# ruanjinchen/Point-Cloud-Flow-Matching

Measured on AMD Instinct MI355X. Metric: train-step points/sec (B=8, N=20000, xyz+rgb) at 1/2/4/8 MI355X; Chamfer ms, higher is better.
Workload: dtype fp32 ContextNet (scatter/gather ops fp32; Conv3d + 1x1 convs as bf16x3 split-operand matrix-core products, fp32 accumulate, ~2^-16 per product vs the reference's default cuDNN TF32 2^-11) + bf16 autocast per-point MLP head (reference AMP config; its per-cloud B-row layers -- embeddings, FiLM affines

## Files before the change

### point-cloud-flow-matching_amd/csrc/head_film.hip

```cpp
#include <algorithm>

#include "pcfm_common.hpp"

namespace pcfm {
namespace {

#ifndef PCFM_FILM_BWD_WPE
#define PCFM_FILM_BWD_WPE 0
#endif
#if PCFM_FILM_BWD_WPE > 0
#define FILM_BWD_ATTR __attribute__((amdgpu_waves_per_eu(PCFM_FILM_BWD_WPE)))
#else
#define FILM_BWD_ATTR
#endif
constexpr int kRowsPerBlock = 256;
constexpr int kSums = 5;

__device__ __forceinline__ float bf2f(uint32_t b) { return __uint_as_float(b << 16); }
__device__ __forceinline__ uint32_t f2bf(float x) {
  return (uint32_t)__builtin_bit_cast(uint16_t, (__bf16)x);
}

__device__ __forceinline__ float wave_sum(float x) {
#pragma unroll
  for (int off = 32; off > 0; off >>= 1) x += __shfl_xor(x, off, 64);
  return x;
}

template <int NV>
__device__ __forceinline__ void ld_f32(const float* __restrict__ p, int lane, float (&v)[NV][4]) {
#pragma unroll
  for (int j = 0; j < NV; ++j) {
    const float4 f = *reinterpret_cast<const float4*>(p + 256 * j + 4 * lane);
    v[j][0] = f.x;
    v[j][1] = f.y;
    v[j][2] = f.z;
    v[j][3] = f.w;
  }
}

template <int NV>
__device__ __forceinline__ void ld_bf16(const uint16_t* __restrict__ p, int lane,
                                        float (&v)[NV][4]) {
#pragma unroll
  for (int j = 0; j < NV; ++j) {
    const uint2 q = *reinterpret_cast<const uint2*>(p + 256 * j + 4 * lane);
    v[j][0] = bf2f(q.x & 0xFFFFu);
    v[j][1] = bf2f(q.x >> 16);
    v[j][2] = bf2f(q.y & 0xFFFFu);
    v[j][3] = bf2f(q.y >> 16);
  }
}

template <int NV>
__device__ __forceinline__ void st_f32(float* __restrict__ p, int lane, const float (&v)[NV][4]) {
#pragma unroll
  for (int j = 0; j < NV; ++j)
    *reinterpret_cast<float4*>(p + 256 * j + 4 * lane) =
        make_float4(v[j][0], v[j][1], v[j][2], v[j][3]);
}

template <int NV>
__device__ __forceinline__ void st_bf16(uint16_t* __restrict__ p, int lane,
                                        const float (&v)[NV][4]) {
#pragma unroll
  for (int j = 0; j < NV; ++j) {
    uint2 q;
    q.x = f2bf(v[j][0]) | (f2bf(v[j][1]) << 16);
    q.y = f2bf(v[j][2]) | (f2bf(v[j][3]) << 16);
// ... 163 lines not shown
                       sh[j][e];
      }
#pragma unroll
      for (int j = 0; j < NV; ++j)
#pragma unroll
        for (int e = 0; e < 4; ++e) {
          const float d = du[j][e] + da[j][e] * dsilu(uu[j][e]);
          const float xc = rstd * (x[j][e] - mean);
          const float y = __builtin_fmaf(gm[j][e], xc, bt[j][e]);
          const float dy = d * sp[j][e];
          acc[0][j][e] += d * y;
          acc[1][j][e] += d;
          acc[2][j][e] += dy * xc;
          acc[3][j][e] += dy;
          xh[j][e] = xc;
          dxh[j][e] = dy * gm[j][e];
          s1 += dxh[j][e];
          s2 += dxh[j][e] * xc;
        }
      const float m1 = wave_sum(s1) * (1.0f / W), m2 = wave_sum(s2) * (1.0f / W);
#pragma unroll
      for (int j = 0; j < NV; ++j)
#pragma unroll
        for (int e = 0; e < 4; ++e) g[j][e] = rstd * (dxh[j][e] - m1 - xh[j][e] * m2);
    } else {
#pragma unroll
      for (int j = 0; j < NV; ++j)
#pragma unroll
        for (int e = 0; e < 4; ++e) g[j][e] = da[j][e] * dsilu(x[j][e]);
    }
    if (dh != nullptr) st_f32<NV>(dh + off, lane, g);
    st_bf16<NV>(dh16 + off, lane, g);
#pragma unroll
    for (int j = 0; j < NV; ++j)
#pragma unroll
      for (int e = 0; e < 4; ++e) acc[4][j][e] += bf2f(f2bf(g[j][e]));
  }
  __syncthreads();
#pragma unroll
  for (int k = 0; k < kSums; ++k)
#pragma unroll
    for (int j = 0; j < NV; ++j)
#pragma unroll
      for (int e = 0; e < 4; ++e) red[wave][k][256 * j + 4 * lane + e] = acc[k][j][e];
  __syncthreads();
  float* pb = part + ((size_t)b * gridDim.x + blockIdx.x) * kSums * W;
  for (int idx = threadIdx.x; idx < kSums * W; idx += 256) {
    const int k = idx / W, c = idx - k * W;
    pb[idx] = ((red[0][k][c] + red[1][k][c]) + red[2][k][c]) + red[3][k][c];
  }
}

__global__ void __launch_bounds__(256)
    film_bwd_reduce_kernel(const float* __restrict__ part, int B, int chunks, int W,
                           float* __restrict__ dsp1, float* __restrict__ dshift,
                           float* __restrict__ perb) {
  __shared__ float red[4][64];
  const int cl = threadIdx.x & 63, grp = threadIdx.x >> 6;
  const int c = blockIdx.x * 64 + cl, k = blockIdx.y, b = blockIdx.z;
  float s = 0.0f;
  if (c < W) {
    const float* p = part + ((size_t)b * chunks * kSums + k) * W + c;
    int q = grp;
    for (; q + 12 < chunks; q += 16) {
      float v[4];
#pragma unroll
      for (int u = 0; u < 4; ++u) v[u] = p[(size_t)(q + 4 * u) * kSums * W];
#pragma unroll
      for (int u = 0; u < 4; ++u) s += v[u];
    }
    for (; q < chunks; q += 4) s += p[(size_t)q * kSums * W];
  }
  red[grp][cl] = s;
  __syncthreads();
  if (grp != 0 || c >= W) return;
  s = ((red[0][cl] + red[1][cl]) + red[2][cl]) + red[3][cl];
  float* out = k == 0 ? dsp1 : k == 1 ? dshift : perb + (size_t)(k - 2) * B * W;
  if (out != nullptr) out[(size_t)b * W + c] = s;
}

__global__ void __launch_bounds__(64)
    film_bwd_reduce2_kernel(const float* __restrict__ perb, int B, int W,
                            float* __restrict__ dgamma, float* __restrict__ dbeta,
                            float* __restrict__ dbias) {
  const int c = blockIdx.x * 64 + threadIdx.x, k = blockIdx.y;
  float* out = k == 0 ? dgamma : k == 1 ? dbeta : dbias;
  if (c >= W || out == nullptr) return;
  float s = 0.0f;
  for (int b = 0; b < B; ++b) s += perb[((size_t)k * B + b) * W + c];
  out[c] = s;
}

int film_fwd_rows() {
  const char* e = getenv("PCFM_FILM_FWD_ROWS");
  const int v = e != nullptr ? atoi(e) : 32;
  return v >= 4 && v % 4 == 0 ? v : 32;
}

bool film_ok(int b, int n, int w) {
  return b > 0 && n > 0 && (w == 256 || w == 512) &&
         (long long)b * n * w < (1LL << 40);
}

template <bool FILM>
int launch_fwd(const void* h16, const float* uprev, const void* gprev, const float* gamma,
               const float* beta, const void* sp1, const void* shift, const float* hbias, int b,
               int n, int w, float eps, float* u, void* a, float* mean, float* rstd,
               hipStream_t st) {
  const int rpb = film_fwd_rows();
  const dim3 grid(ceil_div(n, rpb), b), blk(256);
  const uint16_t* H = (const uint16_t*)h16;
  const uint16_t* G = (const uint16_t*)gprev;
  const uint16_t* S1 = (const uint16_t*)sp1;
  const uint16_t* SH = (const uint16_t*)shift;
  uint16_t* A = (uint16_t*)a;
  switch (w) {
    case 256:
      hipLaunchKernelGGL((film_fwd_kernel<1, FILM>), grid, blk, 0, st, H, uprev, G, gamma, beta,
                         S1, SH, hbias, n, eps, u, A, mean, rstd, rpb);
      break;
    default:
      hipLaunchKernelGGL((film_fwd_kernel<2, FILM>), grid, blk, 0, st, H, uprev, G, gamma, beta,
                         S1, SH, hbias, n, eps, u, A, mean, rstd, rpb);
  }
  return check_launch(FILM ? "head_film_fwd" : "head_silu_fwd");
}

template <bool FILM>
int launch_bwd(const float* dhn, const void* da16, const float* u, const void* h16,
               const float* uprev, const void* gprev, const float* mean, const float* rstd,
               const float* gamma, const float* beta, const void* sp1, const void* shift,
               const float* hbias, int b, int n, int w, float* dh, void* dh16, float* dsp1, float* dshift, float* dgamma,
               float* dbeta, float* dbias, float* dbias_b, void* ws, hipStream_t st) {
  const int chunks = ceil_div(n, kRowsPerBlock);
  const dim3 grid(chunks, b), blk(256);
  const uint16_t* DA = (const uint16_t*)da16;
  const uint16_t* H = (const uint16_t*)h16;
  const uint16_t* G = (const uint16_t*)gprev;
  const uint16_t* S1 = (const uint16_t*)sp1;
  const uint16_t* SH = (const uint16_t*)shift;
  uint16_t* D16 = (uint16_t*)dh16;
  float* part = (float*)ws;
  switch (w) {
    case 256:
      hipLaunchKernelGGL((film_bwd_kernel<1, FILM>), grid, blk, 0, st, dhn, DA, u, H, uprev, G,
                         mean, rstd, gamma, beta, S1, SH, hbias, n, dh, D16, part);
      break;
    default:
      hipLaunchKernelGGL((film_bwd_kernel<2, FILM>), grid, blk, 0, st, dhn, DA, u, H, uprev, G,
                         mean, rstd, gamma, beta, S1, SH, hbias, n, dh, D16, part);
  }
  float* perb = part + (size_t)b * chunks * kSums * w;
  hipLaunchKernelGGL(film_bwd_reduce_kernel, dim3(ceil_div(w, 64), kSums, b), dim3(256), 0, st,
                     (const float*)part, b, chunks, w, dsp1, dshift, perb);
  hipLaunchKernelGGL(film_bwd_reduce2_kernel, dim3(ceil_div(w, 64), 3), dim3(64), 0, st,
                     (const float*)perb, b, w, dgamma, dbeta, dbias);
  if (dbias_b != nullptr) {
    const hipError_t e = hipMemcpyAsync(dbias_b, perb + 2 * (size_t)b * w,
                                        (size_t)b * w * sizeof(float), hipMemcpyDeviceToDevice, st);
    if (e != hipSuccess) {
      set_error("head_film_bwd: hipMemcpyAsync: %s", hipGetErrorString(e));
      return (int)e;
    }
  }
  return check_launch(FILM ? "head_film_bwd" : "head_silu_bwd");
}

}
}

using namespace pcfm;

extern "C" int pcfm_head_film_fwd(const void* h16, const float* hbias, const float* uprev,
                                  const void* gprev, const float* gamma, const float* beta,
                                  const void* sp1, const void* shift, int b, int n, int w,
                                  float eps, float* u, void* a, float* mean, float* rstd,
                                  void* stream) {
  PCFM_CHECK_ARG(film_ok(b, n, w), "head_film_fwd: bad shape b=%d n=%d w=%d", b, n, w);
  PCFM_CHECK_ARG(h16 != nullptr || (uprev != nullptr && gprev != nullptr),
                 "head_film_fwd: need h16 or (uprev, gprev)");
  return launch_fwd<true>(h16, uprev, gprev, gamma, beta, sp1, shift,
                          h16 != nullptr ? hbias : nullptr, b, n, w, eps, u, a, mean, rstd,
                          (hipStream_t)stream);
}

extern "C" int pcfm_head_silu_fwd(const float* uprev, const void* gprev, int b, int n, int w,
                                  void* a, void* stream) {
  PCFM_CHECK_ARG(film_ok(b, n, w), "head_silu_fwd: bad shape b=%d n=%d w=%d", b, n, w);
  return launch_fwd<false>(nullptr, uprev, gprev, nullptr, nullptr, nullptr, nullptr, nullptr, b,
                           n, w, 0.0f, nullptr, a, nullptr, nullptr, (hipStream_t)stream);
}

extern "C" size_t pcfm_head_bwd_workspace_bytes(int b, int n, int w) {
  if (!film_ok(b, n, w)) return 0;
  return ((size_t)b * ceil_div(n, kRowsPerBlock) * kSums + 3 * (size_t)b) * w * sizeof(float);
}

extern "C" int pcfm_head_film_bwd(const float* dh_next, const void* da16, const float* u,
                                  const void* h16, const float* hbias, const float* uprev,
                                  const void* gprev, const float* mean, const float* rstd,
                                  const float* gamma, const float* beta, const void* sp1,
                                  const void* shift, int b, int n, int w, float* dh, void* dh16,
                                  float* dsp1, float* dshift,
                                  float* dgamma, float* dbeta, float* dbias, float* dbias_b,
                                  void* ws, size_t ws_bytes, void* stream) {
  PCFM_CHECK_ARG(film_ok(b, n, w), "head_film_bwd: bad shape b=%d n=%d w=%d", b, n, w);
  PCFM_CHECK_ARG(h16 != nullptr || (uprev != nullptr && gprev != nullptr),
                 "head_film_bwd: need h16 or (uprev, gprev)");
  PCFM_CHECK_ARG(u != nullptr || shift != nullptr, "head_film_bwd: need u or shift");
  PCFM_CHECK_ARG(ws_bytes >= pcfm_head_bwd_workspace_bytes(b, n, w),
                 "head_film_bwd: workspace %zu < %zu bytes", ws_bytes,
                 pcfm_head_bwd_workspace_bytes(b, n, w));
  return launch_bwd<true>(dh_next, da16, u, h16, uprev, gprev, mean, rstd, gamma, beta, sp1, shift,
                          h16 != nullptr ? hbias : nullptr, b, n, w, dh, dh16, dsp1, dshift,
                          dgamma, dbeta, dbias, dbias_b, ws, (hipStream_t)stream);
}

extern "C" int pcfm_head_silu_bwd(const void* da16, const float* uprev, const void* gprev, int b,
                                  int n, int w, float* dh, void* dh16, float* dbias, void* ws,
                                  size_t ws_bytes, void* stream) {
  PCFM_CHECK_ARG(film_ok(b, n, w), "head_silu_bwd: bad shape b=%d n=%d w=%d", b, n, w);
  PCFM_CHECK_ARG(ws_bytes >= pcfm_head_bwd_workspace_bytes(b, n, w),
                 "head_silu_bwd: workspace %zu < %zu bytes", ws_bytes,
                 pcfm_head_bwd_workspace_bytes(b, n, w));
  return launch_bwd<false>(nullptr, da16, nullptr, nullptr, uprev, gprev, nullptr, nullptr,
                           nullptr, nullptr, nullptr, nullptr, nullptr, b, n, w, dh, dh16, nullptr,
                           nullptr, nullptr, nullptr, dbias, nullptr, ws, (hipStream_t)stream);
}
```

### point-cloud-flow-matching_amd/pcfm/_lib.py

```python
from __future__ import annotations

import ctypes
import os
import threading

_HERE = os.path.dirname(os.path.abspath(__file__))
LIB_PATH = os.path.join(os.path.dirname(_HERE), "csrc", "libpcfm_hip.so")
LIB_PATH = os.environ.get("PCFM_LIB", LIB_PATH)

_P = ctypes.c_void_p
_I = ctypes.c_int
_F = ctypes.c_float
_Z = ctypes.c_size_t
_L = ctypes.c_longlong
_D = ctypes.c_double
_DP = ctypes.POINTER(ctypes.c_double)

SIGNATURES = {
    "pcfm_abi_version": (_I, []),
    "pcfm_last_error": (ctypes.c_char_p, []),
    "pcfm_avg_voxelize_fwd_workspace_bytes": (_Z, [_I, _I, _I, _I]),
    "pcfm_avg_voxelize_fwd": (_I, [_P, _P, _I, _I, _I, _I, _P, _P, _P, _P, _Z, _P]),
    "pcfm_avg_voxelize_bwd": (_I, [_P, _P, _P, _I, _I, _I, _I, _P, _P]),
    "pcfm_trilinear_devoxelize_fwd": (_I, [_P, _P, _I, _I, _I, _I, _I, _P, _P, _P, _P]),
# ... 89 lines not shown
                             _P]),
    "pcfm_bn_act_fwd_split": (_I, [_P, _P, _P, _I, _I, _I, _F, _F, _F, _P, _P, _P, _P, _P, _P,
                                   _P, _Z, _P]),
    "pcfm_bn_act_bwd_split_workspace_bytes": (_Z, [_I, _I, _I]),
    "pcfm_bn_act_bwd_split": (_I, [_P, _P, _P, _P, _P, _P, _I, _I, _I, _F, _P, _P, _P, _P, _P,
                                   _Z, _P]),
    "pcfm_gn_film_workspace_bytes": (_Z, [_I, _I, _I, _I]),
    "pcfm_gn_film_res_fwd": (_I, [_P, _P, _P, _P, _P, _I, _I, _I, _I, _F, _P, _P, _P, _P, _Z,
                                  _P]),
    "pcfm_gn_film_res_bwd": (_I, [_P, _P, _P, _P, _P, _P, _P, _I, _I, _I, _I, _P, _P, _P, _P,
                                  _P, _P, _Z, _P]),
    "pcfm_debug_devox_verify_bn": (_I, [_P, _P, _P, _P, _P, _P, _F, _P, _P, _P, _P, _P, _P, _F,
                                        _P, _P, _P, _I, _I, _I, _I, _P, _P]),
    "pcfm_gn_film_res_fwd_bnin": (_I, [_P, _P, _P, _P, _P, _F, _P, _P, _P, _P, _I, _I, _I, _I,
                                       _F, _P, _P, _P, _P, _Z, _P]),
    "pcfm_gn_bnin_parts": (_I, [_I, _I]),
    "pcfm_gn_film_res_bwd_bnin": (_I, [_P, _P, _P, _P, _P, _P, _F, _P, _P, _P, _P, _P, _I, _I,
                                       _I, _I, _P, _P, _P, _P, _P, _P, _P, _Z, _P]),
    "pcfm_bn_act_bwd_apply_parts": (_I, [_P, _P, _P, _P, _P, _P, _P, _I, _I, _I, _I, _F, _P, _P,
                                         _P, _P, _P, _Z, _P]),
    "pcfm_seg_plan_bytes": (_Z, [_I, _I, _I, _I]),
    "pcfm_seg_apply_workspace_bytes": (_Z, [_I, _I, _I, _I, _I]),
    "pcfm_avg_voxelize_plan": (_I, [_P, _I, _I, _I, _P, _P, _P, _Z, _P]),
    "pcfm_avg_voxelize_fwd_planned": (_I, [_P, _P, _I, _I, _I, _I, _P, _P, _Z, _P]),
    "pcfm_trilinear_devoxelize_bwd_plan": (_I, [_P, _P, _I, _I, _I, _P, _Z, _P]),
    "pcfm_trilinear_devoxelize_bwd_planned": (_I, [_P, _P, _I, _I, _I, _I, _P, _P, _Z, _P]),
    "pcfm_adamw_chunk_elems": (_I, []),
    "pcfm_adamw_workspace_bytes": (_Z, [_I]),
    "pcfm_adamw_grad_norm": (_I, [_P, _I, _P, _I, _P, _F, _P, _P, _P, _Z, _P]),
    "pcfm_adamw_ema_step": (_I, [_P, _P, _I, _P, _P, _I, _DP, _DP, _D, _D, _D, _D, _P]),
}

ABI_VERSION = 20

ND_SIGNATURES = {
    "pcfm_chamfer_nd_abi_version": (_I, []),
    "pcfm_chamfer_nd_supported": (_I, [_I]),
    "pcfm_chamfer_nd_workspace_bytes": (_Z, [_I, _I, _I, _I]),
    "pcfm_chamfer_nd_fwd": (_I, [_P, _P, _I, _I, _I, _I, _P, _P, _P, _P, _P, _Z, _P]),
    "pcfm_chamfer_nd_bwd": (_I, [_P, _P, _I, _I, _I, _I, _P, _P, _P, _P, _P, _P, _P]),
}

ND_ABI_VERSION = 1

CROSS_SIGNATURES = {
    "pcfm_chamfer_cross_abi_version": (_I, []),
    "pcfm_chamfer_cross_supported": (_I, [_I]),
    "pcfm_chamfer_cross_workspace_bytes": (_Z, [_I, _I, _I, _I, _I]),
    "pcfm_chamfer_cross_fwd": (_I, [_P, _P, _I, _I, _I, _I, _I, _P, _P, _P, _Z, _P]),
}

CROSS_ABI_VERSION = 1

_lock = threading.Lock()
_lib = None


class PcfmError(RuntimeError):
    """A pcfm_* entry point returned a non-zero status."""


def load() -> ctypes.CDLL:
    global _lib
    if _lib is not None:
        return _lib
    with _lock:
        if _lib is None:
            if not os.path.exists(LIB_PATH):
                raise RuntimeError(
                    f"pcfm: HIP library {LIB_PATH} is not built; run "
                    "`python -c 'import __graft_entry__ as g; g.build()'` "
                    "(HIP tensors have no fallback)")
            lib = ctypes.CDLL(LIB_PATH)
            for table in (SIGNATURES, ND_SIGNATURES, CROSS_SIGNATURES):
                for name, (res, args) in table.items():
                    fn = getattr(lib, name)
                    fn.restype = res
                    fn.argtypes = args
            v = lib.pcfm_abi_version()
            if v != ABI_VERSION:
                raise RuntimeError(f"pcfm: ABI version {v} != expected {ABI_VERSION}; rebuild")
            v = lib.pcfm_chamfer_nd_abi_version()
            if v != ND_ABI_VERSION:
                raise RuntimeError(f"pcfm: chamfer_nd ABI version {v} != expected "
                                   f"{ND_ABI_VERSION}; rebuild")
            v = lib.pcfm_chamfer_cross_abi_version()
            if v != CROSS_ABI_VERSION:
                raise RuntimeError(f"pcfm: chamfer_cross ABI version {v} != expected "
                                   f"{CROSS_ABI_VERSION}; rebuild")
            _lib = lib
    return _lib


def call(name: str, *args) -> None:
    lib = load()
    rc = getattr(lib, name)(*args)
    if rc != 0:
        msg = lib.pcfm_last_error().decode(errors="replace")
        raise PcfmError(f"{name} failed (status {rc}): {msg}")


def query(name: str, *args) -> int:
    return int(getattr(load(), name)(*args))
```

### point-cloud-flow-matching_amd/pcfm/layers.py

```python
from __future__ import annotations

import os

import torch
import torch.nn as nn
import torch.nn.functional as F

__all__ = ["RowsLinear"]


class _RowsLinearBF16(torch.autograd.Function):
    @staticmethod
    def forward(ctx, x, w, b):
        ctx.save_for_backward(x, w)
        ctx.has_bias = b is not None
        return F.linear(x, w, b)

    @staticmethod
    def backward(ctx, gy):
        from pcfm import ops
        x, w = ctx.saved_tensors
        lead = gy.shape[:-1]
        g2 = gy.reshape(-1, gy.shape[-1])
        if g2.stride(1) != 1:
            g2 = g2.contiguous()
        gx = gw = gb = None
        if ctx.needs_input_grad[0]:
            gx = torch.mm(g2, w).view(*lead, w.shape[1])
        if ctx.needs_input_grad[1]:
            x2 = x.reshape(-1, x.shape[-1])
            if x2.stride(1) != 1:
                x2 = x2.contiguous()
            gw = ops.rows_wgrad_bf16(g2, x2)
        if ctx.has_bias and ctx.needs_input_grad[2]:
            gb = ops.rows_colsum(g2).to(g2.dtype) if ops.colsum_ok(g2) else g2.sum(0)
        return gx, gw, gb


class RowsLinear(nn.Linear):

    def forward(self, x: torch.Tensor) -> torch.Tensor:
        if (x.is_cuda and torch.is_autocast_enabled("cuda")
                and torch.get_autocast_dtype("cuda") == torch.bfloat16
                and x.numel() // max(1, x.shape[-1]) >= 4096):
            dt = torch.bfloat16
            b = self.bias.to(dt) if self.bias is not None else None
            with torch.autocast("cuda", enabled=False):
                return _RowsLinearBF16.apply(x.to(dt), self.weight.to(dt), b)
        return super().forward(x)


_PER_BLOCK = 6


class _HeadTrunkBF16(torch.autograd.Function):
    @staticmethod
    def forward(ctx, n, eps, x16, w_in, hb, w_out, b_out, *blk):
        from pcfm import ops
        nb = len(blk) // _PER_BLOCK
        h1 = F.linear(x16, w_in)
        hb = hb.contiguous()
        us, gs, as_, stats = [], [], [], []
        u = g = None
        for k in range(nb):
            lw, lb, sp1, sh, wk, bk = blk[_PER_BLOCK * k:_PER_BLOCK * (k + 1)]
            u, a, mean, rstd = ops.head_film_fwd(h1 if k == 0 else None, u, g, lw, lb, sp1, sh,
                                                 n, eps, hbias=hb if k == 0 else None)
            g = F.linear(a, wk, bk)
            us.append(u)
            gs.append(g)
            as_.append(a)
            stats += [mean, rstd]
        a_out = ops.head_silu_fwd(u, g, n)
        out = F.linear(a_out, w_out, b_out)
        ctx.n, ctx.eps, ctx.nb = n, eps, nb
        ctx.save_for_backward(x16, w_in, h1, hb, w_out, a_out, *us, *gs, *as_, *stats, *blk)
        return out

    @staticmethod
    def backward(ctx, gout):
        from pcfm import ops
        n, nb = ctx.n, ctx.nb
        sv = ctx.saved_tensors
        x16, w_in, h1, hb, w_out, a_out = sv[:6]
        us, gs, as_ = sv[6:6 + nb], sv[6 + nb:6 + 2 * nb], sv[6 + 2 * nb:6 + 3 * nb]
        stats = sv[6 + 3 * nb:6 + 5 * nb]
        blk = sv[6 + 5 * nb:]
        gout = gout.contiguous()
        d_w_out = ops.rows_wgrad_bf16(gout, a_out)
        d_b_out = ops.rows_colsum(gout).to(gout.dtype) if ops.colsum_ok(gout) else gout.sum(0)
        da = torch.mm(gout, w_out)
        dh, dh16, dbias = ops.head_silu_bwd(da, us[-1], gs[-1], n)
        d_blk = [None] * len(blk)
        for k in range(nb - 1, -1, -1):
            lw, lb, sp1, sh, wk, _ = blk[_PER_BLOCK * k:_PER_BLOCK * (k + 1)]
            d_blk[_PER_BLOCK * k + 4] = ops.rows_wgrad_bf16(dh16, as_[k])
            d_blk[_PER_BLOCK * k + 5] = dbias.to(torch.bfloat16)
            da = torch.mm(dh16, wk)
            first = k == 0
            res = ops.head_film_bwd(
                dh, da, None, h1 if first else None, None if first else us[k - 1],
                None if first else gs[k - 1], stats[2 * k], stats[2 * k + 1], lw, lb, sp1, n,
                want_dh=not first, hbias=hb if first else None, shift=sh)
            dh, dh16, dsp1, dshift, dgamma, dbeta, dbias = res[:7]
            if first:
                d_hb = res[7]
            d_blk[_PER_BLOCK * k] = dgamma
            d_blk[_PER_BLOCK * k + 1] = dbeta
            d_blk[_PER_BLOCK * k + 2] = dsp1.to(torch.bfloat16)
            d_blk[_PER_BLOCK * k + 3] = dshift.to(torch.bfloat16)
        d_w_in = ops.rows_wgrad_bf16(dh16, x16)
        dx = torch.mm(dh16, w_in)
        return (None, None, dx, d_w_in, d_hb, d_w_out, d_b_out, *d_blk)


def fused_trunk_supported(trunk, h: torch.Tensor, emb: torch.Tensor, n: int) -> bool:
    if not (h.is_cuda and h.dim() == 2 and torch.is_autocast_enabled("cuda")
            and torch.get_autocast_dtype("cuda") == torch.bfloat16):
        return False
    if getattr(trunk, "film_per_point", False) or emb.dim() != 2 or emb.shape[0] * n != h.shape[0]:
        return False
    width = trunk.input.out_features
    if len(trunk.films) == 0 or width not in (256, 512) or trunk.input.bias is None or trunk.out[1].bias is None:
        return False
    for seq, film in zip(trunk.blocks, trunk.films):
        norm = film.norm
        if not (isinstance(norm, nn.LayerNorm) and norm.elementwise_affine
                and norm.weight is not None and norm.bias is not None
                and tuple(norm.normalized_shape) == (width,)) or seq[1].bias is None:
            return False
    eps = {film.norm.eps for film in trunk.films}
    return len(eps) <= 1


_FILM_BATCH = os.environ.get("PCFM_FILM_BATCH", "1") != "0"


def fused_trunk(trunk, h: torch.Tensor, emb: torch.Tensor, n: int) -> torch.Tensor:
    dt = torch.bfloat16
    blk = []
    from pcfm.models import _batch_fp32
    ctx, fp32 = _batch_fp32(emb)
    nb = len(trunk.films)
    if fp32 and nb > 1 and _FILM_BATCH:
        with ctx:
# ... 57 lines not shown
```

### point-cloud-flow-matching_amd/pcfm/ops.py

```python
from __future__ import annotations

import ctypes
import types

import torch

from . import _lib, cpu_ops


def _check_cuda(x: torch.Tensor, name: str) -> None:
    if not (isinstance(x, torch.Tensor) and x.is_cuda):
        raise RuntimeError(f"{name} must be a CUDA tensor")


def _check_contig(x: torch.Tensor, name: str) -> None:
    if not x.is_contiguous():
        raise RuntimeError(f"{name} must be a contiguous tensor")


def _check_float(x: torch.Tensor, name: str) -> None:
    if x.dtype != torch.float32:
        raise RuntimeError(f"{name} must be a float tensor")


# ... 1042 lines not shown
        _lib.call("pcfm_head_film_fwd", _p(h16), _p(hbias), _p(uprev), _p(gprev), _p(gamma),
                  _p(beta),
                  _p(sp1), _p(shift), b, n, w, float(eps), _p(u), _p(a), _p(mean), _p(rstd),
                  _stream(ref))
    return u, a, mean, rstd


def head_silu_fwd(uprev, gprev, n: int):
    rows, w = uprev.shape
    a = torch.empty((rows, w), dtype=torch.bfloat16, device=uprev.device)
    _lib.call("pcfm_head_silu_fwd", _p(uprev), _p(gprev), rows // n, n, w, _p(a),
              _stream(uprev))
    return a


def head_film_bwd(dh_next, da16, u, h16, uprev, gprev, mean, rstd, gamma, beta, sp1, n: int,
                  want_dh: bool, hbias=None, shift=None):
    rows, w = da16.shape
    b = rows // n
    dev = da16.device
    dh = torch.empty((rows, w), dtype=torch.float32, device=dev) if want_dh else None
    dh16 = torch.empty((rows, w), dtype=torch.bfloat16, device=dev)
    small = torch.empty((3 * b + 3, w), dtype=torch.float32, device=dev)
    dsp1, dshift = small[:b], small[b:2 * b]
    dgamma, dbeta, dbias = small[2 * b], small[2 * b + 1], small[2 * b + 2]
    dbias_b = small[2 * b + 3:] if hbias is not None else None
    ws = _workspace(_lib.query("pcfm_head_bwd_workspace_bytes", b, n, w), da16)
    if u is None and shift is None:
        raise ValueError("head_film_bwd: need u or shift")
    with _timed("head_film_bwd", rows * w * (4 + 2 + (4 if u is not None else 0)
                                             + (2 if h16 is not None else 6)
                                             + (4 if want_dh else 0) + 2), da16):
        _lib.call("pcfm_head_film_bwd", _p(dh_next), _p(da16), _p(u), _p(h16), _p(hbias),
                  _p(uprev), _p(gprev), _p(mean), _p(rstd), _p(gamma), _p(beta), _p(sp1),
                  _p(shift), b, n,
                  w, _p(dh), _p(dh16), _p(dsp1), _p(dshift), _p(dgamma), _p(dbeta), _p(dbias),
                  _p(dbias_b), _p(ws), ws.numel(), _stream(da16))
    if hbias is not None:
        return dh, dh16, dsp1, dshift, dgamma, dbeta, dbias, dbias_b
    return dh, dh16, dsp1, dshift, dgamma, dbeta, dbias


def head_silu_bwd(da16, uprev, gprev, n: int):
    rows, w = da16.shape
    b = rows // n
    dev = da16.device
    dh = torch.empty((rows, w), dtype=torch.float32, device=dev)
    dh16 = torch.empty((rows, w), dtype=torch.bfloat16, device=dev)
    dbias = torch.empty((w,), dtype=torch.float32, device=dev)
    ws = _workspace(_lib.query("pcfm_head_bwd_workspace_bytes", b, n, w), da16)
    _lib.call("pcfm_head_silu_bwd", _p(da16), _p(uprev), _p(gprev), b, n, w, _p(dh), _p(dh16),
              _p(dbias), _p(ws), ws.numel(), _stream(da16))
    return dh, dh16, dbias


def _counter(t, like: torch.Tensor):
    if t is None:
        return None
    if t.dtype != torch.int64 or t.numel() != 1 or t.device != like.device:
        raise RuntimeError("num_batches_tracked: expected a one-element int64 tensor on the "
                           "input's device")
    return t


def bn_act_forward(x: torch.Tensor, weight: torch.Tensor, bias: torch.Tensor, eps: float,
                   slope: float, momentum: float, running_mean, running_var,
                   num_batches_tracked=None):
    _check(x, "input", "f")
    b, c = x.shape[0], x.shape[1]
    s = x.numel() // max(1, b * c)
    y = torch.empty_like(x)
    stats = torch.empty((2, c), dtype=torch.float32, device=x.device)
    ws = _workspace(_lib.query("pcfm_bn_workspace_bytes", b, c, s), x)
    with _timed("bn_act_fwd", 4 * 3 * x.numel(), x):
        _lib.call("pcfm_bn_act_fwd", _ptr(x), _ptr(weight), _ptr(bias), b, c, s, float(eps),
                  float(slope), float(momentum), _p(running_mean), _p(running_var),
                  _p(_counter(num_batches_tracked, x)), _ptr(y),
                  _ptr(stats[0]), _ptr(stats[1]), _ptr(ws), ws.numel(), _stream(x))
    return y, stats[0], stats[1]


def bn_act_forward_parts(x: torch.Tensor, stats: torch.Tensor, weight: torch.Tensor,
                         bias: torch.Tensor, eps: float, slope: float, momentum: float,
                         running_mean, running_var, num_batches_tracked=None):
    _check(x, "input", "f")
    _check(stats, "stats", "f")
    b, c = x.shape[0], x.shape[1]
    s = x.numel() // max(1, b * c)
    y = torch.empty_like(x)
    out = torch.empty((2, c), dtype=torch.float32, device=x.device)
    with _timed("bn_act_fwd", 4 * 2 * x.numel(), x):
        _lib.call("pcfm_bn_act_fwd_parts", _ptr(x), _ptr(stats), int(stats.shape[1]),
                  _ptr(weight), _ptr(bias), b, c, s, float(eps), float(slope), float(momentum),
                  _p(running_mean), _p(running_var), _p(_counter(num_batches_tracked, x)),
                  _ptr(y), _ptr(out[0]), _ptr(out[1]), _stream(x))
    return y, out[0], out[1]


def bn_act_forward_split(x: torch.Tensor, weight: torch.Tensor, bias: torch.Tensor, eps: float,
                         slope: float, momentum: float, running_mean, running_var,
                         num_batches_tracked=None):
    _check(x, "input", "f")
    b, c, r = x.shape[0], x.shape[1], x.shape[2]
    s = x.numel() // max(1, b * c)
    n = _lib.query("pcfm_conv3d_split_bytes", b, c, r)
    if n == 0 or c % 64 != 0:
# ... 320 lines not shown
```

Baseline: 5.712 million.

## Fuse head SiLU with narrow output linear in forward and backward kernels

Adds HIP kernels that compute SiLU of the last trunk activation and apply the small (up to 8 outputs) output linear in one pass, using cross-lane permlane/DPP reductions. The backward fuses the grad of the output linear (dW, db, da) with the SiLU backward and the bias column sum. The existing two-stage reduction is generalised to a variable number of sums. This avoids materialising the bf16 activation a_out, the separate GEMM launches, and the extra wgrad/colsum passes. In exchange it adds per-kind partial workspaces and a more register-heavy backward kernel.

Result: no change. 5.751 million (median of 6 runs) (+0.7%).

```diff
diff --git a/include/pcfm_head_out.h b/include/pcfm_head_out.h
--- /dev/null
+++ b/include/pcfm_head_out.h
@@ -0,0 +1,30 @@
+#ifndef PCFM_HEAD_OUT_H
+#define PCFM_HEAD_OUT_H
+
+#include <stddef.h>
+
+#ifdef __cplusplus
+extern "C" {
+#endif
+
+#define PCFM_HEAD_OUT_ABI_VERSION 1
+#define PCFM_HEAD_OUT_MAX 8
+
+int pcfm_head_out_abi_version(void);
+
+int pcfm_head_silu_out_fwd(const float* uprev, const void* gprev, const void* w_out,
+                           const void* b_out, int b, int n, int w, int n_out, void* out,
+                           void* stream);
+
+size_t pcfm_head_silu_out_bwd_workspace_bytes(int b, int n, int w, int n_out);
+
+int pcfm_head_silu_out_bwd(const void* gout, const float* uprev, const void* gprev,
+                           const void* w_out, int b, int n, int w, int n_out, float* dh,
+                           void* dh16, float* dw, float* db, float* dbias, void* ws,
+                           size_t ws_bytes, void* stream);
+
+#ifdef __cplusplus
+}
+#endif
+
+#endif
diff --git a/point-cloud-flow-matching_amd/csrc/head_film.hip b/point-cloud-flow-matching_amd/csrc/head_film.hip
--- a/point-cloud-flow-matching_amd/csrc/head_film.hip
+++ b/point-cloud-flow-matching_amd/csrc/head_film.hip
@@ -1,5 +1,6 @@
 #include <algorithm>
 
+#include "../../include/pcfm_head_out.h"
 #include "pcfm_common.hpp"
 
 namespace pcfm {
@@ -15,6 +16,8 @@
 #endif
 constexpr int kRowsPerBlock = 256;
 constexpr int kSums = 5;
+constexpr int kOutMax = PCFM_HEAD_OUT_MAX;
+constexpr int kMaxKinds = kOutMax + 2;
 
 __device__ __forceinline__ float bf2f(uint32_t b) { return __uint_as_float(b << 16); }
 __device__ __forceinline__ uint32_t f2bf(float x) {
@@ -284,43 +287,229 @@
 }
 
 __global__ void __launch_bounds__(256)
-    film_bwd_reduce_kernel(const float* __restrict__ part, int B, int chunks, int W,
-                           float* __restrict__ dsp1, float* __restrict__ dshift,
+    film_bwd_reduce_kernel(const float* __restrict__ part, int B, int chunks, int W, int nk,
+                           int nb, float* __restrict__ dsp1, float* __restrict__ dshift,
                            float* __restrict__ perb) {
   __shared__ float red[4][64];
   const int cl = threadIdx.x & 63, grp = threadIdx.x >> 6;
   const int c = blockIdx.x * 64 + cl, k = blockIdx.y, b = blockIdx.z;
+  const size_t step = (size_t)nk * W;
   float s = 0.0f;
   if (c < W) {
-    const float* p = part + ((size_t)b * chunks * kSums + k) * W + c;
+    const float* p = part + ((size_t)b * chunks * nk + k) * W + c;
     int q = grp;
     for (; q + 12 < chunks; q += 16) {
       float v[4];
 #pragma unroll
-      for (int u = 0; u < 4; ++u) v[u] = p[(size_t)(q + 4 * u) * kSums * W];
+      for (int u = 0; u < 4; ++u) v[u] = p[(size_t)(q + 4 * u) * step];
 #pragma unroll
       for (int u = 0; u < 4; ++u) s += v[u];
     }
-    for (; q < chunks; q += 4) s += p[(size_t)q * kSums * W];
+    for (; q < chunks; q += 4) s += p[(size_t)q * step];
   }
   red[grp][cl] = s;
   __syncthreads();
   if (grp != 0 || c >= W) return;
   s = ((red[0][cl] + red[1][cl]) + red[2][cl]) + red[3][cl];
-  float* out = k == 0 ? dsp1 : k == 1 ? dshift : perb + (size_t)(k - 2) * B * W;
+  float* out = k >= nb ? perb + (size_t)(k - nb) * B * W : k == 0 ? dsp1 : dshift;
   if (out != nullptr) out[(size_t)b * W + c] = s;
 }
 
+struct Stage2 {
+  float* out[kMaxKinds];
+  int cols[kMaxKinds];
+};
+
 __global__ void __launch_bounds__(64)
-    film_bwd_reduce2_kernel(const float* __restrict__ perb, int B, int W,
-                            float* __restrict__ dgamma, float* __restrict__ dbeta,
-                            float* __restrict__ dbias) {
+    film_bwd_reduce2_kernel(const float* __restrict__ perb, int B, int W, Stage2 to) {
   const int c = blockIdx.x * 64 + threadIdx.x, k = blockIdx.y;
-  float* out = k == 0 ? dgamma : k == 1 ? dbeta : dbias;
-  if (c >= W || out == nullptr) return;
+  float* out = to.out[k];
+  if (c >= to.cols[k] || out == nullptr) return;
   float s = 0.0f;
   for (int b = 0; b < B; ++b) s += perb[((size_t)k * B + b) * W + c];
   out[c] = s;
+}
+
+
+__device__ __forceinline__ float swap_add32(float a, float b) {
+  const auto r =
+      __builtin_amdgcn_permlane32_swap(__float_as_uint(a), __float_as_uint(b), false, false);
+  return __uint_as_float(r[0]) + __uint_as_float(r[1]);
+}
+__device__ __forceinline__ float swap_add16(float a, float b) {
+  const auto r =
+      __builtin_amdgcn_permlane16_swap(__float_as_uint(a), __float_as_uint(b), false, false);
+  return __uint_as_float(r[0]) + __uint_as_float(r[1]);
+}
+template <int N>
+__device__ __forceinline__ float ror_add(float x) {
+  return x + __int_as_float(
+                 __builtin_amdgcn_update_dpp(0, __float_as_int(x), 0x120 + N, 0xf, 0xf, false));
+}
+
+template <int P>
+__device__ __forceinline__ void wave_sum_cols(float (&p)[P]) {
+  constexpr int M1 = P > 1 ? P / 2 : 1, M2 = M1 > 1 ? M1 / 2 : 1;
+#pragma unroll
+  for (int i = 0; i < M1; ++i) p[i] = swap_add32(p[i], p[P > 1 ? i + M1 : i]);
+#pragma unroll
+  for (int i = 0; i < M2; ++i) p[i] = swap_add16(p[i], p[M1 > 1 ? i + M2 : i]);
+#pragma unroll
+  for (int i = 0; i < M2; ++i) p[i] = ror_add<1>(ror_add<2>(ror_add<4>(ror_add<8>(p[i]))));
+}
+
+constexpr int pow2_ge(int x) { return x <= 1 ? 1 : x <= 2 ? 2 : x <= 4 ? 4 : 8; }
+
+template <int NV>
+struct RawRow {
+  float4 u[NV];
+  uint2 g[NV];
+};
+template <int NV>
+__device__ __forceinline__ void ld_raw(const float* __restrict__ uprev,
+                                       const uint16_t* __restrict__ gprev, size_t off, int lane,
+                                       RawRow<NV>& r) {
+#pragma unroll
+  for (int j = 0; j < NV; ++j) {
+    r.u[j] = *reinterpret_cast<const float4*>(uprev + off + 256 * j + 4 * lane);
+    r.g[j] = *reinterpret_cast<const uint2*>(gprev + off + 256 * j + 4 * lane);
+  }
+}
+template <int NV>
+__device__ __forceinline__ void h_of_raw(const RawRow<NV>& r, float (&x)[NV][4]) {
+#pragma unroll
+  for (int j = 0; j < NV; ++j) {
+    x[j][0] = r.u[j].x + bf2f(r.g[j].x & 0xFFFFu);
+    x[j][1] = r.u[j].y + bf2f(r.g[j].x >> 16);
+    x[j][2] = r.u[j].z + bf2f(r.g[j].y & 0xFFFFu);
+    x[j][3] = r.u[j].w + bf2f(r.g[j].y >> 16);
+  }
+}
+
+template <int NV, int OUT>
+__global__ void __launch_bounds__(256)
+    silu_out_fwd_kernel(const float* __restrict__ uprev, const uint16_t* __restrict__ gprev,
+                        const uint16_t* __restrict__ wout, const uint16_t* __restrict__ bout,
+                        int n, uint16_t* __restrict__ out, int rpb) {
+  constexpr int W = 256 * NV, P = pow2_ge(OUT);
+  constexpr int M1 = P > 1 ? P / 2 : 1, M2 = M1 > 1 ? M1 / 2 : 1;
+  const int lane = threadIdx.x & 63, wave = threadIdx.x >> 6;
+  const int b = blockIdx.y;
+  const int i0 = blockIdx.x * rpb, i1 = min(n, i0 + rpb);
+  float wr[OUT][NV][4];
+#pragma unroll
+  for (int j = 0; j < OUT; ++j) ld_bf16<NV>(wout + (size_t)j * W, lane, wr[j]);
+  const int h5 = lane >> 5, h4 = (lane >> 4) & 1, li = lane & 15;
+  int jl = li;
+  bool holder = li < M2;
+  if (M1 > 1) jl += M2 * h4; else holder = holder && h4 == 0;
+  if (P > 1) jl += M1 * h5; else holder = holder && h5 == 0;
+  holder = holder && jl < OUT;
+  const float bj = holder && bout != nullptr ? bf2f(bout[jl]) : 0.0f;
+  for (int i = i0 + wave; i < i1; i += 4) {
+    const size_t row = (size_t)b * n + i;
+    RawRow<NV> raw;
+    ld_raw<NV>(uprev, gprev, row * W, lane, raw);
+    float x[NV][4];
+    h_of_raw<NV>(raw, x);
+    float p[P];
+#pragma unroll
+    for (int j = 0; j < P; ++j) p[j] = 0.0f;
+#pragma unroll
+    for (int jj = 0; jj < NV; ++jj)
+#pragma unroll
+      for (int e = 0; e < 4; ++e) {
+        const float a = bf2f(f2bf(silu(x[jj][e])));
+#pragma unroll
+        for (int j = 0; j < OUT; ++j) p[j] = __builtin_fmaf(a, wr[j][jj][e], p[j]);
+      }
+    wave_sum_cols<P>(p);
+    const float t = M2 > 1 && li == 1 ? p[M2 - 1] : p[0];
+    if (holder) out[row * OUT + jl] = (uint16_t)f2bf(bj + t);
+  }
+}
+
+template <int NV>
+__device__ __forceinline__ void block_partial(float (*red)[256 * NV], int wave, int lane,
+                                              const float (&v)[NV][4],
+                                              float* __restrict__ pbk) {
+  __syncthreads();
+  st_f32<NV>(red[wave], lane, v);
+  __syncthreads();
+  for (int c = threadIdx.x; c < 256 * NV; c += 256)
+    pbk[c] = ((red[0][c] + red[1][c]) + red[2][c]) + red[3][c];
+}
+
+template <int NV, int OUT>
+__global__ void __launch_bounds__(256)
+    silu_out_bwd_kernel(const uint16_t* __restrict__ gout, const float* __restrict__ uprev,
+                        const uint16_t* __restrict__ gprev, const uint16_t* __restrict__ wout,
+                        int n, float* __restrict__ dh, uint16_t* __restrict__ dh16,
+                        float* __restrict__ part) {
+  constexpr int W = 256 * NV;
+  __shared__ float wl[OUT][W];
+  __shared__ float red[4][W];
+  const int lane = threadIdx.x & 63, wave = threadIdx.x >> 6;
+  const int b = blockIdx.y;
+  const int i0 = blockIdx.x * kRowsPerBlock, i1 = min(n, i0 + kRowsPerBlock);
+  for (int idx = threadIdx.x; idx < OUT * W; idx += 256) (&wl[0][0])[idx] = bf2f(wout[idx]);
+  __syncthreads();
+  float acc[OUT + 1][NV][4], db[OUT];
+#pragma unroll
+  for (int k = 0; k <= OUT; ++k)
+#pragma unroll
+    for (int j = 0; j < NV; ++j)
+#pragma unroll
+      for (int e = 0; e < 4; ++e) acc[k][j][e] = 0.0f;
+#pragma unroll
+  for (int j = 0; j < OUT; ++j) db[j] = 0.0f;
+#pragma nounroll
+  for (int i = i0 + wave; i < i1; i += 4) {
+    const size_t row = (size_t)b * n + i;
+    const size_t off = row * W;
+    asm volatile("" ::: "memory");
+    RawRow<NV> raw;
+    uint16_t gr[OUT];
+    ld_raw<NV>(uprev, gprev, off, lane, raw);
+#pragma unroll
+    for (int j = 0; j < OUT; ++j) gr[j] = gout[row * OUT + j];
+    float go[OUT], x[NV][4], g[NV][4];
+#pragma unroll
+    for (int j = 0; j < OUT; ++j) go[j] = bf2f(gr[j]);
+    h_of_raw<NV>(raw, x);
+#pragma unroll
+    for (int j = 0; j < OUT; ++j) db[j] += go[j];
+#pragma unroll
+    for (int jj = 0; jj < NV; ++jj) {
+      float da[4] = {0.0f, 0.0f, 0.0f, 0.0f};
+#pragma unroll
+      for (int j = 0; j < OUT; ++j) {
+        const float4 wv = *reinterpret_cast<const float4*>(&wl[j][256 * jj + 4 * lane]);
+        da[0] = __builtin_fmaf(go[j], wv.x, da[0]);
+        da[1] = __builtin_fmaf(go[j], wv.y, da[1]);
+        da[2] = __builtin_fmaf(go[j], wv.z, da[2]);
+        da[3] = __builtin_fmaf(go[j], wv.w, da[3]);
+      }
+#pragma unroll
+      for (int e = 0; e < 4; ++e) {
+        const float a = bf2f(f2bf(silu(x[jj][e])));
+#pragma unroll
+        for (int j = 0; j < OUT; ++j) acc[j][jj][e] = __builtin_fmaf(go[j], a, acc[j][jj][e]);
+        g[jj][e] = bf2f(f2bf(da[e])) * dsilu(x[jj][e]);
+        acc[OUT][jj][e] += bf2f(f2bf(g[jj][e]));
+      }
+    }
+    if (dh != nullptr) st_f32<NV>(dh + off, lane, g);
+    st_bf16<NV>(dh16 + off, lane, g);
+  }
+  float* pb = part + ((size_t)b * gridDim.x + blockIdx.x) * (OUT + 2) * W;
+#pragma unroll
+  for (int k = 0; k <= OUT; ++k) block_partial<NV>(red, wave, lane, acc[k], pb + (size_t)k * W);
+  float v[NV][4] = {};
+#pragma unroll
+  for (int q = 0; q < OUT; ++q)
+    if (lane == q / 4) v[0][q % 4] = db[q];
+  block_partial<NV>(red, wave, lane, v, pb + (size_t)(OUT + 1) * W);
 }
 
 int film_fwd_rows() {
@@ -384,9 +573,12 @@
   }
   float* perb = part + (size_t)b * chunks * kSums * w;
   hipLaunchKernelGGL(film_bwd_reduce_kernel, dim3(ceil_div(w, 64), kSums, b), dim3(256), 0, st,
-                     (const float*)part, b, chunks, w, dsp1, dshift, perb);
+                     (const float*)part, b, chunks, w, kSums, 2, dsp1, dshift, perb);
+  Stage2 to = {};
+  to.out[0] = dgamma, to.out[1] = dbeta, to.out[2] = dbias;
+  to.cols[0] = to.cols[1] = to.cols[2] = w;
   hipLaunchKernelGGL(film_bwd_reduce2_kernel, dim3(ceil_div(w, 64), 3), dim3(64), 0, st,
-                     (const float*)perb, b, w, dgamma, dbeta, dbias);
+                     (const float*)perb, b, w, to);
   if (dbias_b != nullptr) {
     const hipError_t e = hipMemcpyAsync(dbias_b, perb + 2 * (size_t)b * w,
                                         (size_t)b * w * sizeof(float), hipMemcpyDeviceToDevice, st);
@@ -397,6 +589,37 @@
   }
   return check_launch(FILM ? "head_film_bwd" : "head_silu_bwd");
 }
+
+bool out_ok(int b, int n, int w, int n_out) {
+  return film_ok(b, n, w) && n_out >= 1 && n_out <= kOutMax;
+}
+
+template <int NV, int OUT>
+void launch_out_fwd(const float* uprev, const uint16_t* G, const uint16_t* Wo, const uint16_t* Bo,
+                    int b, int n, uint16_t* out, hipStream_t st) {
+  const int rpb = film_fwd_rows();
+  hipLaunchKernelGGL((silu_out_fwd_kernel<NV, OUT>), dim3(ceil_div(n, rpb), b), dim3(256), 0, st,
+                     uprev, G, Wo, Bo, n, out, rpb);
+}
+
+template <int NV, int OUT>
+void launch_out_bwd(const uint16_t* GO, const float* uprev, const uint16_t* G, const uint16_t* Wo,
+                    int b, int n, float* dh, uint16_t* dh16, float* part, hipStream_t st) {
+  hipLaunchKernelGGL((silu_out_bwd_kernel<NV, OUT>), dim3(ceil_div(n, kRowsPerBlock), b),
+                     dim3(256), 0, st, GO, uprev, G, Wo, n, dh, dh16, part);
+}
+
+#define PCFM_OUT_CASES(fn, nv, ...)          \
+  switch (n_out) {                           \
+    case 1: fn<nv, 1>(__VA_ARGS__); break;   \
+    case 2: fn<nv, 2>(__VA_ARGS__); break;   \
+    case 3: fn<nv, 3>(__VA_ARGS__); break;   \
+    case 4: fn<nv, 4>(__VA_ARGS__); break;   \
+    case 5: fn<nv, 5>(__VA_ARGS__); break;   \
+    case 6: fn<nv, 6>(__VA_ARGS__); break;   \
+    case 7: fn<nv, 7>(__VA_ARGS__); break;   \
+    default: fn<nv, 8>(__VA_ARGS__);         \
+  }
 
 }
 }
@@ -459,3 +682,70 @@
                            nullptr, nullptr, nullptr, nullptr, nullptr, b, n, w, dh, dh16, nullptr,
                            nullptr, nullptr, nullptr, dbias, nullptr, ws, (hipStream_t)stream);
 }
+
+extern "C" int pcfm_head_out_abi_version(void) { return PCFM_HEAD_OUT_ABI_VERSION; }
+
+extern "C" int pcfm_head_silu_out_fwd(const float* uprev, const void* gprev, const void* w_out,
+                                      const void* b_out, int b, int n, int w, int n_out,
+                                      void* out, void* stream) {
+  PCFM_CHECK_ARG(out_ok(b, n, w, n_out), "head_silu_out_fwd: bad shape b=%d n=%d w=%d n_out=%d",
+                 b, n, w, n_out);
+  PCFM_CHECK_ARG(uprev != nullptr && gprev != nullptr && w_out != nullptr && out != nullptr,
+                 "head_silu_out_fwd: null uprev, gprev, w_out or out");
+  const uint16_t* G = (const uint16_t*)gprev;
+  const uint16_t* Wo = (const uint16_t*)w_out;
+  const uint16_t* Bo = (const uint16_t*)b_out;
+  uint16_t* O = (uint16_t*)out;
+  hipStream_t st = (hipStream_t)stream;
+  if (w == 256) {
+    PCFM_OUT_CASES(launch_out_fwd, 1, uprev, G, Wo, Bo, b, n, O, st)
+  } else {
+    PCFM_OUT_CASES(launch_out_fwd, 2, uprev, G, Wo, Bo, b, n, O, st)
+  }
+  return check_launch("head_silu_out_fwd");
+}
+
+extern "C" size_t pcfm_head_silu_out_bwd_workspace_bytes(int b, int n, int w, int n_out) {
+  if (!out_ok(b, n, w, n_out)) return 0;
+  return ((size_t)b * ceil_div(n, kRowsPerBlock) + (size_t)b) * (n_out + 2) * w * sizeof(float);
+}
+
+extern "C" int pcfm_head_silu_out_bwd(const void* gout, const float* uprev, const void* gprev,
+                                      const void* w_out, int b, int n, int w, int n_out,
+                                      float* dh, void* dh16, float* dw, float* db, float* dbias,
+                                      void* ws, size_t ws_bytes, void* stream) {
+  PCFM_CHECK_ARG(out_ok(b, n, w, n_out), "head_silu_out_bwd: bad shape b=%d n=%d w=%d n_out=%d",
+                 b, n, w, n_out);
+  PCFM_CHECK_ARG(gout != nullptr && uprev != nullptr && gprev != nullptr && w_out != nullptr &&
+                     dh16 != nullptr,
+                 "head_silu_out_bwd: null gout, uprev, gprev, w_out or dh16");
+  const size_t need = pcfm_head_silu_out_bwd_workspace_bytes(b, n, w, n_out);
+  PCFM_CHECK_ARG(ws != nullptr && ws_bytes >= need, "head_silu_out_bwd: workspace %zu < %zu bytes",
+                 ws_bytes, need);
+  const uint16_t* GO = (const uint16_t*)gout;
+  const uint16_t* G = (const uint16_t*)gprev;
+  const uint16_t* Wo = (const uint16_t*)w_out;
+  uint16_t* D16 = (uint16_t*)dh16;
+  hipStream_t st = (hipStream_t)stream;
+  const int chunks = ceil_div(n, kRowsPerBlock), nk = n_out + 2;
+  float* part = (float*)ws;
+  if (w == 256) {
+    PCFM_OUT_CASES(launch_out_bwd, 1, GO, uprev, G, Wo, b, n, dh, D16, part, st)
+  } else {
+    PCFM_OUT_CASES(launch_out_bwd, 2, GO, uprev, G, Wo, b, n, dh, D16, part, st)
+  }
+  float* perb = part + (size_t)b * chunks * nk * w;
+  hipLaunchKernelGGL(film_bwd_reduce_kernel, dim3(ceil_div(w, 64), nk, b), dim3(256), 0, st,
+                     (const float*)part, b, chunks, w, nk, 0, (float*)nullptr, (float*)nullptr,
+                     perb);
+  Stage2 to = {};
+  for (int j = 0; j < n_out; ++j) {
+    to.out[j] = dw != nullptr ? dw + (size_t)j * w : nullptr;
+    to.cols[j] = w;
+  }
+  to.out[n_out] = dbias, to.cols[n_out] = w;
+  to.out[n_out + 1] = db, to.cols[n_out + 1] = n_out;
+  hipLaunchKernelGGL(film_bwd_reduce2_kernel, dim3(ceil_div(w, 64), nk), dim3(64), 0, st,
+                     (const float*)perb, b, w, to);
+  return check_launch("head_silu_out_bwd");
+}
diff --git a/point-cloud-flow-matching_amd/pcfm/_lib.py b/point-cloud-flow-matching_amd/pcfm/_lib.py
--- a/point-cloud-flow-matching_amd/pcfm/_lib.py
+++ b/point-cloud-flow-matching_amd/pcfm/_lib.py
@@ -165,6 +165,16 @@
 
 CROSS_ABI_VERSION = 1
 
+HEAD_OUT_SIGNATURES = {
+    "pcfm_head_out_abi_version": (_I, []),
+    "pcfm_head_silu_out_fwd": (_I, [_P, _P, _P, _P, _I, _I, _I, _I, _P, _P]),
+    "pcfm_head_silu_out_bwd_workspace_bytes": (_Z, [_I, _I, _I, _I]),
+    "pcfm_head_silu_out_bwd": (_I, [_P, _P, _P, _P, _I, _I, _I, _I, _P, _P, _P, _P, _P, _P, _Z,
+                                    _P]),
+}
+
+HEAD_OUT_ABI_VERSION = 1
+
 _lock = threading.Lock()
 _lib = None
 
@@ -185,7 +195,7 @@
                     "`python -c 'import __graft_entry__ as g; g.build()'` "
                     "(HIP tensors have no fallback)")
             lib = ctypes.CDLL(LIB_PATH)
-            for table in (SIGNATURES, ND_SIGNATURES, CROSS_SIGNATURES):
+            for table in (SIGNATURES, ND_SIGNATURES, CROSS_SIGNATURES, HEAD_OUT_SIGNATURES):
                 for name, (res, args) in table.items():
                     fn = getattr(lib, name)
                     fn.restype = res
@@ -201,6 +211,10 @@
             if v != CROSS_ABI_VERSION:
                 raise RuntimeError(f"pcfm: chamfer_cross ABI version {v} != expected "
                                    f"{CROSS_ABI_VERSION}; rebuild")
+            v = lib.pcfm_head_out_abi_version()
+            if v != HEAD_OUT_ABI_VERSION:
+                raise RuntimeError(f"pcfm: head_out ABI version {v} != expected "
+                                   f"{HEAD_OUT_ABI_VERSION}; rebuild")
             _lib = lib
     return _lib
 
diff --git a/point-cloud-flow-matching_amd/pcfm/layers.py b/point-cloud-flow-matching_amd/pcfm/layers.py
--- a/point-cloud-flow-matching_amd/pcfm/layers.py
+++ b/point-cloud-flow-matching_amd/pcfm/layers.py
@@ -51,6 +51,8 @@
 
 
 _PER_BLOCK = 6
+_HEAD_OUT_FUSED = os.environ.get("PCFM_HEAD_OUT_FUSED", "1") != "0"
+_HEAD_OUT_MAX = 8
 
 
 class _HeadTrunkBF16(torch.autograd.Function):
@@ -71,10 +73,16 @@
             gs.append(g)
             as_.append(a)
             stats += [mean, rstd]
-        a_out = ops.head_silu_fwd(u, g, n)
-        out = F.linear(a_out, w_out, b_out)
-        ctx.n, ctx.eps, ctx.nb = n, eps, nb
-        ctx.save_for_backward(x16, w_in, h1, hb, w_out, a_out, *us, *gs, *as_, *stats, *blk)
+        fused_out = _HEAD_OUT_FUSED and w_out.shape[0] <= _HEAD_OUT_MAX
+        if fused_out:
+            out = ops.head_silu_out_fwd(u, g, w_out, b_out, n)
+            last = ()
+        else:
+            a_out = ops.head_silu_fwd(u, g, n)
+            out = F.linear(a_out, w_out, b_out)
+            last = (a_out,)
+        ctx.n, ctx.eps, ctx.nb, ctx.fused_out = n, eps, nb, fused_out
+        ctx.save_for_backward(x16, w_in, h1, hb, w_out, *last, *us, *gs, *as_, *stats, *blk)
         return out
 
     @staticmethod
@@ -82,15 +90,21 @@
         from pcfm import ops
         n, nb = ctx.n, ctx.nb
         sv = ctx.saved_tensors
-        x16, w_in, h1, hb, w_out, a_out = sv[:6]
-        us, gs, as_ = sv[6:6 + nb], sv[6 + nb:6 + 2 * nb], sv[6 + 2 * nb:6 + 3 * nb]
-        stats = sv[6 + 3 * nb:6 + 5 * nb]
-        blk = sv[6 + 5 * nb:]
+        x16, w_in, h1, hb, w_out = sv[:5]
+        o = 5 if ctx.fused_out else 6
+        us, gs, as_ = sv[o:o + nb], sv[o + nb:o + 2 * nb], sv[o + 2 * nb:o + 3 * nb]
+        stats = sv[o + 3 * nb:o + 5 * nb]
+        blk = sv[o + 5 * nb:]
         gout = gout.contiguous()
-        d_w_out = ops.rows_wgrad_bf16(gout, a_out)
-        d_b_out = ops.rows_colsum(gout).to(gout.dtype) if ops.colsum_ok(gout) else gout.sum(0)
-        da = torch.mm(gout, w_out)
-        dh, dh16, dbias = ops.head_silu_bwd(da, us[-1], gs[-1], n)
+        if ctx.fused_out:
+            dh, dh16, dbias, d_w_out, d_b_out = ops.head_silu_out_bwd(gout, us[-1], gs[-1], w_out, n)
+            d_w_out, d_b_out = d_w_out.to(torch.bfloat16), d_b_out.to(torch.bfloat16)
+        else:
+            a_out = sv[5]
+            d_w_out = ops.rows_wgrad_bf16(gout, a_out)
+            d_b_out = ops.rows_colsum(gout).to(gout.dtype) if ops.colsum_ok(gout) else gout.sum(0)
+            da = torch.mm(gout, w_out)
+            dh, dh16, dbias = ops.head_silu_bwd(da, us[-1], gs[-1], n)
         d_blk = [None] * len(blk)
         for k in range(nb - 1, -1, -1):
             lw, lb, sp1, sh, wk, _ = blk[_PER_BLOCK * k:_PER_BLOCK * (k + 1)]
diff --git a/point-cloud-flow-matching_amd/pcfm/ops.py b/point-cloud-flow-matching_amd/pcfm/ops.py
--- a/point-cloud-flow-matching_amd/pcfm/ops.py
+++ b/point-cloud-flow-matching_amd/pcfm/ops.py
@@ -1118,6 +1118,54 @@
     _lib.call("pcfm_head_silu_bwd", _p(da16), _p(uprev), _p(gprev), b, n, w, _p(dh), _p(dh16),
               _p(dbias), _p(ws), ws.numel(), _stream(da16))
     return dh, dh16, dbias
+
+
+HEAD_OUT_MAX = 8
+
+
+def _head_out_weight(w_out, w: int, name: str):
+    if (w_out.dtype != torch.bfloat16 or w_out.dim() != 2 or w_out.shape[1] != w
+            or not 1 <= w_out.shape[0] <= HEAD_OUT_MAX):
+        raise RuntimeError(f"{name}: w_out must be bf16 (n_out <= {HEAD_OUT_MAX}, {w}), got "
+                           f"{w_out.dtype} {tuple(w_out.shape)}")
+    return w_out.contiguous()
+
+
+def head_silu_out_fwd(uprev, gprev, w_out, b_out, n: int):
+    rows, w = uprev.shape
+    w_out = _head_out_weight(w_out, w, "head_silu_out_fwd")
+    n_out = w_out.shape[0]
+    if b_out is not None:
+        if b_out.dtype != torch.bfloat16 or b_out.shape != (n_out,):
+            raise RuntimeError("head_silu_out_fwd: b_out must be bf16 (n_out,)")
+        b_out = b_out.contiguous()
+    out = torch.empty((rows, n_out), dtype=torch.bfloat16, device=uprev.device)
+    with _timed("head_silu_out_fwd", rows * w * 6 + rows * n_out * 2, uprev):
+        _lib.call("pcfm_head_silu_out_fwd", _p(uprev), _p(gprev), _p(w_out), _p(b_out),
+                  rows // n, n, w, n_out, _p(out), _stream(uprev))
+    return out
+
+
+def head_silu_out_bwd(gout, uprev, gprev, w_out, n: int):
+    rows, w = uprev.shape
+    w_out = _head_out_weight(w_out, w, "head_silu_out_bwd")
+    n_out = w_out.shape[0]
+    if gout.dtype != torch.bfloat16 or gout.shape != (rows, n_out):
+        raise RuntimeError("head_silu_out_bwd: gout must be bf16 (rows, n_out)")
+    gout = gout.contiguous()
+    b = rows // n
+    dev = uprev.device
+    dh = torch.empty((rows, w), dtype=torch.float32, device=dev)
+    dh16 = torch.empty((rows, w), dtype=torch.bfloat16, device=dev)
+    small = torch.empty((n_out + 1, w), dtype=torch.float32, device=dev)
+    dw, dbias = small[:n_out], small[n_out]
+    db = torch.empty((n_out,), dtype=torch.float32, device=dev)
+    ws = _workspace(_lib.query("pcfm_head_silu_out_bwd_workspace_bytes", b, n, w, n_out), uprev)
+    with _timed("head_silu_out_bwd", rows * w * 12 + rows * n_out * 2, uprev):
+        _lib.call("pcfm_head_silu_out_bwd", _p(gout), _p(uprev), _p(gprev), _p(w_out), b, n, w,
+                  n_out, _p(dh), _p(dh16), _p(dw), _p(db), _p(dbias), _p(ws), ws.numel(),
+                  _stream(uprev))
+    return dh, dh16, dbias, dw, db
 
 
 def _counter(t, like: torch.Tensor):
```
